# enoche/MMRec

Hardware: NVIDIA H100
Metric: graph-prop edges/sec (+ full-catalog scored-items/sec in extra) @ d=64 (higher is better)
Workload: dtype f32

## Files before the change

### mmrec_b200/csrc/score_cf.cu

```cuda
#include <climits>
#include <cstdio>
#include <cstdlib>

#include "batch_mask.cuh"
#include "select.cuh"
#include "tc_common.cuh"

namespace mmrec {

using namespace tc;

constexpr int CF_TILE = 128;
constexpr int CF_CONSUMER_WARPS = 8;
constexpr int CF_THREADS = 32 * CF_CONSUMER_WARPS + 32;
constexpr int CF_MAX_STAGES = 10;
constexpr int CF_CAP = 512;
constexpr int CF_EX_SLOTS = 128;
constexpr float CF_EPS = 1.125f / 1024.f;
constexpr float CF_EPS_SUB = 1.0f / 16777216.f;

struct CfSmem {
    uint32_t a, slab0, slab, bars, total;
    int stages;
};
__host__ __device__ inline CfSmem cf_smem(int KP) {
    CfSmem L;
    L.a = 0;
    L.slab0 = 2 * CF_TILE * KP * 2;
    const uint32_t slab = CF_TILE * KP * 2;
    L.slab = slab;
    L.stages = (int)((226u * 1024u - L.slab0 - 300u) / slab);
    if (L.stages > CF_MAX_STAGES) L.stages = CF_MAX_STAGES;
    L.bars = L.slab0 + L.stages * slab;
    L.total = L.bars + 32 * 8;
    return L;
}
enum { CB_AFULL = 0, CB_AFREE = 1, CB_FULL = 2, CB_EMPTY = 2 + CF_MAX_STAGES, CB_END = 2 + 2 * CF_MAX_STAGES };

struct CfParams {
    const char* Upk;
    const char* Ipk;
    int KP, n_it;
    int64_t B, n_items, n_units;
    float* gmax; int G, gw;
    const float* thr; uint4* bitmap;
    int dbg;
};

__device__ __forceinline__ void cf_producer(const CfParams& p, const CfSmem& L, uint32_t sbase, int64_t u0, int64_t u1) {
    const uint32_t bar = sbase + L.bars;
    const uint32_t a_bytes = 2 * CF_TILE * p.KP * 2;
    const uint32_t piece = L.slab < 16384u ? L.slab : 16384u;
    int64_t pair = u0 / p.n_it;
    int it = (int)(u0 - pair * p.n_it);
    bool new_pair = true;
    uint32_t a_cnt = 0, slot = 0, ph = 1;
    for (int64_t u = u0; u < u1; ++u) {
        if (new_pair) {
            if (a_cnt > 0) mbar_wait(bar + CB_AFREE * 8, (a_cnt - 1) & 1);
            mbar_expect_tx(bar + CB_AFULL * 8, a_bytes);
            const char* src = p.Upk + pair * (int64_t)a_bytes;
            for (uint32_t o = 0; o < a_bytes; o += 16384) bulk_g2s(sbase + L.a + o, src + o, 16384, bar + CB_AFULL * 8);
            ++a_cnt;
            new_pair = false;
        }
        const char* src = p.Ipk + (int64_t)it * L.slab;
        const uint32_t fb = bar + (CB_FULL + slot) * 8;
        mbar_wait(bar + (CB_EMPTY + slot) * 8, ph);
        if (p.dbg & 16) {
            mbar_arrive(fb);
        } else {
            mbar_expect_tx(fb, L.slab);
            const uint32_t dst = sbase + L.slab0 + slot * L.slab;
            for (uint32_t o = 0; o < L.slab; o += piece) bulk_g2s(dst + o, src + o, piece, fb);
        }
        if (++slot == (uint32_t)L.stages) { slot = 0; ph ^= 1; }
        if (++it == p.n_it) { it = 0; ++pair; new_pair = true; }
    }
}

template <int PASS, int GPT>
__device__ __forceinline__ void cf_consumer(const CfParams& p, const CfSmem& L, uint32_t sbase, int64_t u0, int64_t u1, int h) {
    const uint32_t bar = sbase + L.bars;
    constexpr uint32_t LBO = (CF_TILE / 8) * 128, SBO = 128;
    const int ksteps = p.KP / 16;
    const uint32_t half_bytes = CF_TILE * p.KP * 2;
    const int t = threadIdx.x & 127, w = t >> 5, lane = t & 31, q = lane & 3;
    const uint64_t a_desc0 = smem_desc(sbase + L.a + h * half_bytes, LBO, SBO), a_desc1 = smem_desc(sbase + L.a + h * half_bytes + 1024, LBO, SBO);
    const uint64_t b_desc0 = smem_desc(sbase + L.slab0, LBO, SBO);
    const uint64_t kstep = (2 * LBO) >> 4;
    const uint64_t slab_step = L.slab >> 4;
    float acc0[64], acc1[64];
#pragma unroll
    for (int i = 0; i < 64; ++i) { acc0[i] = 0.f; acc1[i] = 0.f; }
    int64_t pair = u0 / p.n_it;
    int it = (int)(u0 - pair * p.n_it);
    bool new_pair = true, live = false;
    uint32_t a_cnt = 0, slot = 0, ph = 0;
    uint64_t bd_slot = b_desc0;
    int64_t row0 = 0;
    float thr[4];
    for (int64_t u = u0; u < u1; ++u) {
        if (new_pair) {
            mbar_wait(bar + CB_AFULL * 8, a_cnt & 1);
            ++a_cnt;
            const int64_t base = pair * (2 * CF_TILE) + h * CF_TILE;
            live = base < p.B;
            row0 = base + 16 * w + (lane >> 2);
#pragma unroll
            for (int r = 0; r < 4; ++r) {
                const int64_t rr = row0 + 64 * (r >> 1) + 8 * (r & 1);
                if (PASS == 2) thr[r] = rr < p.B ? __ldg(p.thr + rr) : INFINITY;
            }
            new_pair = false;
        }
        mbar_wait(bar + (CB_FULL + slot) * 8, ph);
        if (live && !(p.dbg & 2)) {
            uint64_t ad0 = a_desc0, ad1 = a_desc1, bd = bd_slot;
            wgmma_fence();
#pragma unroll 4
            for (int j = 0; j < ksteps; ++j) {
                wgmma_f16<CF_TILE>(acc0, ad0, bd, j ? 1u : 0u);
                wgmma_f16<CF_TILE>(acc1, ad1, bd, j ? 1u : 0u);
                ad0 += kstep; ad1 += kstep; bd += kstep;
            }
            wgmma_commit();
            wgmma_wait<0>();
            wgmma_fence_regs(acc0);
            wgmma_fence_regs(acc1);
        }
        warp_arrive(bar + (CB_EMPTY + slot) * 8);
        bd_slot += slab_step;
        if (++slot == (uint32_t)L.stages) { slot = 0; ph ^= 1; bd_slot = b_desc0; }
        const int cur_it = it;
        if (++it == p.n_it) { it = 0; ++pair; new_pair = true; }
        if (new_pair || u + 1 == u1) warp_arrive(bar + CB_AFREE * 8);
        if (!live) continue;
        const int n_valid = (int)(p.n_items - (int64_t)cur_it * CF_TILE);
#pragma unroll
        for (int r = 0; r < 4; ++r) {
            const float* acc = r < 2 ? acc0 : acc1;
            const int e2 = r & 1;
            const int64_t row = row0 + 64 * (r >> 1) + 8 * e2;
            auto val = [&](int j, int e) {
                const float v = acc[4 * j + 2 * e2 + e];
                return 8 * j + 2 * q + e < n_valid ? v : -INFINITY;
            };
            if (PASS == 1) {
                group_max_store<GPT>(r < 2 ? acc0 : acc1, e2, q, n_valid, row, p.B, [&] { return p.gmax + row * p.G + (int64_t)cur_it * GPT; });
            } else {
                uint32_t wd[4] = {0u, 0u, 0u, 0u};
#pragma unroll
                for (int j = 0; j < 16; ++j)
#pragma unroll
                    for (int e = 0; e < 2; ++e)
                        if (!(__float_as_uint(val(j, e) - thr[r]) >> 31)) wd[j >> 2] |= 1u << (31 - (8 * (j & 3) + 2 * q + e));
#pragma unroll
                for (int b = 0; b < 4; ++b) {
                    wd[b] |= __shfl_xor_sync(0xffffffffu, wd[b], 1);
                    wd[b] |= __shfl_xor_sync(0xffffffffu, wd[b], 2);
                }
                if (q == r && row < p.B) p.bitmap[row * p.n_it + cur_it] = make_uint4(wd[0], wd[1], wd[2], wd[3]);
            }
        }
    }
}

template <int PASS, int GPT>
__global__ void __launch_bounds__(CF_THREADS, 1) cf_pass_kernel(const CfParams p) {
    extern __shared__ __align__(1024) uint8_t smem[];
    const CfSmem L = cf_smem(p.KP);
    const uint32_t sbase = smem_u32(smem);
    const int warp = threadIdx.x >> 5, lane = threadIdx.x & 31;
    const uint32_t bar = sbase + L.bars;
    if (threadIdx.x == 0) {
        mbar_init(bar + CB_AFULL * 8, 1);
        mbar_init(bar + CB_AFREE * 8, CF_CONSUMER_WARPS);
        for (int s = 0; s < CF_MAX_STAGES; ++s) {
            mbar_init(bar + (CB_FULL + s) * 8, 1);
            mbar_init(bar + (CB_EMPTY + s) * 8, CF_CONSUMER_WARPS);
        }
        mbar_fence_init();
    }
    __syncthreads();
    const int64_t u0 = (int64_t)blockIdx.x * p.n_units / gridDim.x;
    const int64_t u1 = (int64_t)(blockIdx.x + 1) * p.n_units / gridDim.x;
    if (warp == CF_CONSUMER_WARPS) {
        if (lane == 0) cf_producer(p, L, sbase, u0, u1);
    } else {
        cf_consumer<PASS, GPT>(p, L, sbase, u0, u1, warp >> 2);
    }
}

__device__ __forceinline__ void cf_pack_one(int64_t t, int64_t n_rows, const int64_t* __restrict__ idx, const float* __restrict__ E, int64_t ld,
                                            int d, int KP, const uint32_t* __restrict__ scale_src, uint4* __restrict__ out,
                                            float* __restrict__ row_norm, uint32_t* __restrict__ max_norm) {
    const int kblks = KP / 8;
    const int64_t row = t / kblks;
    const int kb = (int)(t % kblks);
    float x[8];
#pragma unroll
    for (int e = 0; e < 8; ++e) x[e] = 0.f;
    if (row < n_rows) {
        const float* src = E + (idx ? idx[row] : row) * ld;
#pragma unroll
        for (int e = 0; e < 8; ++e)
            if (kb * 8 + e < d) x[e] = __ldg(src + kb * 8 + e);
    }
    uint32_t am = 0u;
    if (!scale_src) {
#pragma unroll
        for (int e = 0; e < 8; ++e) { const uint32_t b = __float_as_uint(x[e]) & 0x7fffffffu; am = b > am ? b : am; }
        for (int o = kblks / 2; o > 0; o >>= 1) {
            const uint32_t a2 = __shfl_xor_sync(0xffffffffu, am, o);
            am = a2 > am ? a2 : am;
        }
    }
    const float sc = fp16_scale_for(scale_src ? __ldg(scale_src) : am);
    float ss = 0.f;
#pragma unroll
    for (int e = 0; e < 8; ++e) ss = fmaf(x[e] * sc, x[e] * sc, ss);
    for (int o = kblks / 2; o > 0; o >>= 1) ss += __shfl_xor_sync(0xffffffffu, ss, o);
    store_fp16x8(out, row / CF_TILE, kblks, kb, (int)(row % CF_TILE), x, sc);
    if (kb == 0 && row < n_rows) {
        const float nrm = sqrtf(ss) * (1.0f + 1e-6f);
        if (row_norm) row_norm[row] = nrm;
        if (max_norm) atomicMax(max_norm, __float_as_uint(nrm));
    }
}

__global__ void __launch_bounds__(256) cf_pack_items_kernel(int64_t n_items, const float* __restrict__ Ie, int64_t ldi, int d, int KP,
                                                            uint4* __restrict__ Ipk, uint32_t* __restrict__ header, int64_t n_threads) {
    const int64_t t = blockIdx.x * (int64_t)blockDim.x + threadIdx.x;
    if (t >= n_threads) return;
    if (t == 0) { header[1] = (uint32_t)n_items; header[2] = (uint32_t)d; header[3] = (uint32_t)KP; }
    cf_pack_one(t, n_items, nullptr, Ie, ldi, d, KP, header + 4, Ipk, nullptr, header);
}

__global__ void __launch_bounds__(256) cf_prep_kernel(int64_t mask_blocks, const BatchMask mask, int64_t nb, const int64_t* __restrict__ users,
                                                      const float* __restrict__ Ue, int64_t ldu, int d, int KP, uint4* __restrict__ Upk,
                                                      float* __restrict__ unorm, int64_t pack_threads, uint32_t* __restrict__ zero, int64_t zero_words) {
    if ((int64_t)blockIdx.x < mask_blocks) {
        mask_sorted_block(blockIdx.x, mask);
        return;
    }
    int64_t t = (blockIdx.x - mask_blocks) * (int64_t)blockDim.x + threadIdx.x;
    if (t < pack_threads) { cf_pack_one(t, nb, users, Ue, ldu, d, KP, nullptr, Upk, unorm, nullptr); return; }
    t -= pack_threads;
    if (t < zero_words) zero[t] = 0;
}

constexpr int CF_THR_BITS = 16;
template <int NV>
__device__ __forceinline__ uint32_t cf_warp_kth_coarse(const float* __restrict__ g, int G, int need, int lane) {
    uint32_t key[NV];
#pragma unroll
    for (int j = 0; j < NV; ++j) {
        const int t = j * 32 + lane;
        key[j] = t < G ? float_key(__ldg(g + t)) : 0u;
    }
    uint32_t kmax = 0u, kmin = 0xffffffffu;
#pragma unroll
    for (int j = 0; j < NV; ++j) {
        kmax = max(kmax, key[j]);
        if (j * 32 + lane < G && key[j] > 0x007fffffu) kmin = min(kmin, key[j]);
    }
    kmax = __reduce_max_sync(0xffffffffu, kmax);
    kmin = __reduce_min_sync(0xffffffffu, kmin);
    const int top = 31 - __clz((kmax ^ kmin) | (1u << (32 - CF_THR_BITS)));
    uint32_t prefix = top >= 31 ? 0u : (kmax & ~((2u << top) - 1u));
#pragma unroll 1
    for (int b = top; b >= 32 - CF_THR_BITS; --b) {
        const uint32_t cand = prefix | (1u << b);
// ... 496 lines not shown
```

### mmrec_b200/csrc/tc_common.cuh

```cuda
#pragma once
#include <cuda_fp16.h>

#include "common.cuh"
#include "wgmma.cuh"

namespace mmrec {
namespace tc {

__device__ __forceinline__ uint32_t smem_u32(const void* p) { return (uint32_t)__cvta_generic_to_shared(p); }

__device__ __forceinline__ void mbar_init(uint32_t bar, uint32_t count) {
    asm volatile("mbarrier.init.shared::cta.b64 [%0], %1;" ::"r"(bar), "r"(count) : "memory");
}
__device__ __forceinline__ void mbar_fence_init() { asm volatile("fence.mbarrier_init.release.cluster;" ::: "memory"); }
__device__ __forceinline__ void mbar_arrive(uint32_t bar) {
    asm volatile("mbarrier.arrive.shared::cta.b64 _, [%0];" ::"r"(bar) : "memory");
}
__device__ __forceinline__ void mbar_expect_tx(uint32_t bar, uint32_t bytes) {
    asm volatile("mbarrier.arrive.expect_tx.shared::cta.b64 _, [%0], %1;" ::"r"(bar), "r"(bytes) : "memory");
}
__device__ __forceinline__ bool mbar_try_wait(uint32_t bar, uint32_t parity) {
    uint32_t ok;
    asm volatile(
        "{\n\t.reg .pred p;\n\t"
        "mbarrier.try_wait.parity.shared::cta.b64 p, [%1], %2;\n\t"
        "selp.u32 %0, 1, 0, p;\n\t}"
        : "=r"(ok) : "r"(bar), "r"(parity) : "memory");
    return ok != 0;
}
__device__ __forceinline__ uint64_t global_ns() {
    uint64_t t;
    asm volatile("mov.u64 %0, %%globaltimer;" : "=l"(t));
    return t;
}
__device__ __forceinline__ void mbar_wait(uint32_t bar, uint32_t parity) {
    uint32_t spins = 0;
    uint64_t t0 = 0;
    while (!mbar_try_wait(bar, parity)) {
        if (++spins == 4096u) t0 = global_ns();
        if (spins > 4096u && (spins & 1023u) == 0 && global_ns() - t0 > 2000000000ull) __trap();
    }
}

__device__ __forceinline__ void bulk_g2s(uint32_t dst_smem, const void* src, uint32_t bytes, uint32_t bar) {
    asm volatile("cp.async.bulk.shared::cluster.global.mbarrier::complete_tx::bytes [%0], [%1], %2, [%3];"
                 ::"r"(dst_smem), "l"(src), "r"(bytes), "r"(bar) : "memory");
}

__device__ __forceinline__ void wgmma_fence() { asm volatile("wgmma.fence.sync.aligned;" ::: "memory"); }
__device__ __forceinline__ void wgmma_commit() { asm volatile("wgmma.commit_group.sync.aligned;" ::: "memory"); }
template <int N>
__device__ __forceinline__ void wgmma_wait() { asm volatile("wgmma.wait_group.sync.aligned %0;" ::"n"(N) : "memory"); }
template <int R>
__device__ __forceinline__ void wgmma_fence_regs(float (&d)[R]) {
#pragma unroll
    for (int i = 0; i < R; ++i) asm volatile("" : "+f"(d[i])::"memory");
}
__device__ __forceinline__ void fence_proxy_async() { asm volatile("fence.proxy.async.shared::cta;" ::: "memory"); }
__device__ __forceinline__ void warp_arrive(uint32_t bar) {
    __syncwarp();
    if ((threadIdx.x & 31) == 0) mbar_arrive(bar);
}

__device__ __forceinline__ uint64_t smem_desc(uint32_t smem_addr, uint32_t lbo_bytes, uint32_t sbo_bytes) {
    uint64_t d = 0;
    d |= (uint64_t)((smem_addr & 0x3FFFFu) >> 4);
    d |= (uint64_t)((lbo_bytes >> 4) & 0x3FFFu) << 16;
    d |= (uint64_t)((sbo_bytes >> 4) & 0x3FFFu) << 32;
    return d;
}

__device__ __forceinline__ void split_tf32(float x, float& hi, float& lo) {
    uint32_t h, l;
    asm("cvt.rna.tf32.f32 %0, %1;" : "=r"(h) : "f"(x));
    hi = __uint_as_float(h);
    asm("cvt.rna.tf32.f32 %0, %1;" : "=r"(l) : "f"(x - hi));
    lo = __uint_as_float(l);
}

__device__ __forceinline__ void split_tf32_trunc(float x, float& hi, float& lo) {
    hi = __uint_as_float(__float_as_uint(x) & 0xffffe000u);
    lo = x - hi;
}

}

__device__ __forceinline__ float fp16_scale_for(uint32_t m_bits) {
    const uint32_t e = (m_bits >> 23) & 0xffu;
    if (e == 0u || e == 255u || e < 14u) return 1.0f;
    return __uint_as_float((268u - e) << 23);
}

__global__ void absmax_norm_kernel(int64_t n, const float* __restrict__ X, int64_t ldx, int F, float* __restrict__ rnorm,
                                   uint32_t* __restrict__ amax, uint32_t* __restrict__ nmax);

__device__ __forceinline__ void store_fp16x8(uint4* __restrict__ out, int64_t tile, int kblks, int kb, int rr, const float (&x)[8], float sc) {
    uint32_t w[4];
#pragma unroll
    for (int e = 0; e < 4; ++e) {
        const __half2 h = __floats2half2_rn(x[2 * e] * sc, x[2 * e + 1] * sc);
        w[e] = *reinterpret_cast<const uint32_t*>(&h);
    }
    out[((tile * kblks + kb) * 16 + rr / 8) * 8 + (rr % 8)] = make_uint4(w[0], w[1], w[2], w[3]);
}

template <int GPT, class Dst>
__device__ __forceinline__ void group_max_store(const float (&acc)[64], int e2, int q, int n_valid, int64_t row, int64_t n_rows, Dst dst) {
    auto val = [&](int j, int e) { return 8 * j + 2 * q + e < n_valid ? acc[4 * j + 2 * e2 + e] : -INFINITY; };
    float gm[GPT];
#pragma unroll
    for (int g = 0; g < GPT; ++g) {
        float m = -INFINITY;
#pragma unroll
        for (int j = g * (16 / GPT); j < (g + 1) * (16 / GPT); ++j) m = fmaxf(m, fmaxf(val(j, 0), val(j, 1)));
        m = fmaxf(m, __shfl_xor_sync(0xffffffffu, m, 1));
        gm[g] = fmaxf(m, __shfl_xor_sync(0xffffffffu, m, 2));
    }
    if (row < n_rows) {
        float* d = dst();
#pragma unroll
        for (int g = 0; g < GPT; ++g)
            if ((g & 3) == q) d[g] = gm[g];
    }
}

__device__ __forceinline__ void set_threshold(float t, float margin, float* thr, int32_t* flag) {
    const bool finite = fabsf(t) < INFINITY && margin < INFINITY;
    *thr = finite ? t - margin : INFINITY;
    *flag = finite ? 0 : 2;
}

constexpr int TC_M = 128;
constexpr int TC_N = 256;
constexpr int TC_KC = 32;
constexpr int TC_SLAB_BYTES = TC_N * TC_KC * 4;
constexpr int TC_THREADS = 288;

template <int R>
__device__ __forceinline__ void pack_split_one(int64_t t, int64_t n_rows, const int64_t* __restrict__ idx, const float* __restrict__ E,
                                               int64_t ld, int d, int KP, float* __restrict__ hi, float* __restrict__ lo) {
    const int kblks = KP / 4;
    const int64_t row = t / kblks;
    const int kb = (int)(t % kblks);
    float x[4] = {0.f, 0.f, 0.f, 0.f};
    if (row < n_rows) {
        const float* src = E + (idx ? idx[row] : row) * ld;
#pragma unroll
        for (int e = 0; e < 4; ++e)
            if (kb * 4 + e < d) x[e] = __ldg(src + kb * 4 + e);
    }
    float4 h, l;
    tc::split_tf32(x[0], h.x, l.x); tc::split_tf32(x[1], h.y, l.y); tc::split_tf32(x[2], h.z, l.z); tc::split_tf32(x[3], h.w, l.w);
    const int64_t tile = row / R;
    const int rr = (int)(row % R);
    const int64_t off = ((tile * kblks + kb) * (R / 8) + rr / 8) * 32 + (rr % 8) * 4;
    *reinterpret_cast<float4*>(hi + off) = h;
    *reinterpret_cast<float4*>(lo + off) = l;
}

template <int R>
__global__ void pack_split_kernel(int64_t n_rows, const int64_t* __restrict__ idx, const float* __restrict__ E, int64_t ld,
                                  int d, int KP, float* __restrict__ hi, float* __restrict__ lo, int64_t n_tiles) {
    const int64_t t = blockIdx.x * (int64_t)blockDim.x + threadIdx.x;
    if (t >= n_tiles * R * (KP / 4)) return;
    pack_split_one<R>(t, n_rows, idx, E, ld, d, KP, hi, lo);
}

}
```

### mmrec_b200/csrc/spmm.cu

```cuda
#include <cooperative_groups.h>

#include "common.cuh"

namespace mmrec {

struct SpmmParams {
    int64_t n_rows, n_cols;
    const int32_t* rowptr; const int32_t* colidx; const float* vals;
    const int4* tasks; int64_t n_tasks, n_heavy; const int4* split_rows; int32_t* counters; float* partial;
    const float* X; int64_t ldx;
    float* Y; int64_t ldy;
    const float* acc_in; float* acc_out; int64_t ldacc; float acc_div;
    const float* gate_ref; int64_t ldgate;
    int y_acc;
    const float* post; int64_t post_row0; uint32_t spost;
    int d;
    uint32_t sx, sy, sacc, sgate;
    const float* X_hi; const float* acc_in_hi;
    int x_split, acc_split;
    uint32_t sx_hi, sacc_hi;
};


__device__ __forceinline__ const float4* row_f4(const float* base, uint32_t stride, int r, int f4) {
// ... 285 lines not shown

template <int D, int T>
__global__ void __launch_bounds__(256, VecCfg<D, T>::V == 1 ? 4 : 0) spmm_vec_kernel(const SpmmParams p) {
    __shared__ __align__(16) float red[(256 / T) * D];
    spmm_vec_body<D, T, false>(p, red);
}

template <int D, int T>
__global__ void __launch_bounds__(256) spmm_drop_kernel(const SpmmParams p, const uint32_t* __restrict__ keep, float scale) {
    __shared__ __align__(16) float red[(256 / T) * D];
    spmm_vec_body<D, T, false, true>(p, red, DropKeep{keep, scale});
}

__global__ void __launch_bounds__(256) edge_keep_bits_kernel(int64_t nnz, const float* __restrict__ draws, float keep_prob,
                                                             const int32_t* __restrict__ draw_of, const int32_t* __restrict__ mirror,
                                                             uint32_t* __restrict__ keep, uint32_t* __restrict__ keep_t) {
    const int64_t n_words = (nnz + 31) >> 5;
    const int lane = threadIdx.x & 31;
    const int64_t w0 = ((int64_t)blockIdx.x * blockDim.x + threadIdx.x) >> 5;
    const int64_t n_warps = ((int64_t)gridDim.x * blockDim.x) >> 5;
    auto kept = [&](int64_t e) { return floorf(__fadd_rn(keep_prob, __ldg(draws + __ldg(draw_of + e)))) != 0.f; };
    for (int64_t w = w0; w < n_words; w += n_warps) {
        const int64_t e = (w << 5) + lane;
        const bool in = e < nnz;
        const uint32_t word = __ballot_sync(0xffffffffu, in && kept(e));
        const uint32_t word_t = keep_t ? __ballot_sync(0xffffffffu, in && kept(__ldg(mirror + e))) : 0u;
        if (lane == 0) {
            keep[w] = word;
            if (keep_t) keep_t[w] = word_t;
        }
    }
}

constexpr int SPMM_CHAIN_MAX = 8;
struct SpmmChain { SpmmParams step[SPMM_CHAIN_MAX]; int n; unsigned sync_mask; };

template <int D, int T, bool COOP>
__global__ void __launch_bounds__(256, 3) spmm_chain_kernel(const SpmmChain c) {
    __shared__ __align__(16) float red[(256 / T) * D];
    for (int i = 0; i < c.n; ++i) {
        if (COOP && ((c.sync_mask >> i) & 1u)) { __threadfence(); cooperative_groups::this_grid().sync(); }
        spmm_vec_body<D, T, true>(c.step[i], red);
    }
}

__global__ void __launch_bounds__(256) spmm_generic_kernel(const SpmmParams p) {
    const int lane = threadIdx.x & 31;
    const int64_t warp0 = (int64_t)blockIdx.x * (blockDim.x >> 5) + (threadIdx.x >> 5);
    const int64_t nwarps = (int64_t)gridDim.x * (blockDim.x >> 5);
    for (int64_t row = warp0; row < p.n_rows; row += nwarps) {
        const int b = p.rowptr[row], e = p.rowptr[row + 1];
        float dot = 0.f, ny = 0.f, nr = 0.f;
        if (p.gate_ref) {
            for (int k0 = 0; k0 < p.d; k0 += 32) {
                const int k = k0 + lane;
                float acc = 0.f;
                if (k < p.d)
                    for (int j = b; j < e; ++j) acc = fmaf(p.vals[j], p.X[(int64_t)p.colidx[j] * p.ldx + k], acc);
                float r = k < p.d ? p.gate_ref[row * p.ldgate + k] : 0.f;
                dot += acc * r; ny += acc * acc; nr += r * r;
            }
            dot = warp_sum(dot); ny = warp_sum(ny); nr = warp_sum(nr);
        }
        const float c = p.gate_ref ? dot / (fmaxf(sqrtf(ny), 1e-8f) * fmaxf(sqrtf(nr), 1e-8f)) : 1.f;
        for (int k0 = 0; k0 < p.d; k0 += 32) {
            const int k = k0 + lane;
            if (k >= p.d) continue;
            float acc = 0.f;
            for (int j = b; j < e; ++j) acc = fmaf(p.vals[j], p.X[(int64_t)p.colidx[j] * p.ldx + k], acc);
            if (p.gate_ref) acc *= c;
            if (p.Y) p.Y[row * p.ldy + k] = p.y_acc ? p.Y[row * p.ldy + k] + acc : acc;
            if (p.acc_out) {
                float a = acc + (p.acc_in ? p.acc_in[row * p.ldacc + k] : 0.f);
                if (p.acc_div != 1.0f) a = __fdiv_rn(a, p.acc_div);
                if (p.post && row >= p.post_row0) a += p.post[(row - p.post_row0) * (int64_t)(p.spost / 4) + k];
                p.acc_out[row * p.ldacc + k] = a;
            }
        }
    }
}

int g_spmm_lanes = 0;

template <int D, int T, bool DROP = false>
static int launch_vec(const SpmmParams& p, cudaStream_t stream, const DropKeep dk = DropKeep{nullptr, 1.f}) {
    static int blocks_per_sm = 0;
    if (!blocks_per_sm) {
        if constexpr (DROP) MMREC_CUDA(cudaOccupancyMaxActiveBlocksPerMultiprocessor(&blocks_per_sm, spmm_drop_kernel<D, T>, 256, 0));
        else MMREC_CUDA(cudaOccupancyMaxActiveBlocksPerMultiprocessor(&blocks_per_sm, spmm_vec_kernel<D, T>, 256, 0));
        if (blocks_per_sm < 1) blocks_per_sm = 1;
    }
    const int64_t n_work = p.tasks ? p.n_tasks : p.n_rows;
    const int per_block = 8 * (32 / T);
    int64_t grid = (n_work - p.n_heavy + per_block - 1) / per_block;
    if (grid < p.n_heavy) grid = p.n_heavy;
    const int64_t cap = (int64_t)sm_count() * blocks_per_sm;
    if (grid > cap) grid = cap;
    if (grid < 1) return MMREC_OK;
    if constexpr (DROP) spmm_drop_kernel<D, T><<<(unsigned)grid, 256, 0, stream>>>(p, dk.keep, dk.scale);
    else spmm_vec_kernel<D, T><<<(unsigned)grid, 256, 0, stream>>>(p);
    MMREC_LAUNCH_CHECK();
    return MMREC_OK;
}

template <int D>
static int launch_vec_d(const SpmmParams& p, cudaStream_t stream) {
    constexpr int T4 = D / 4 > 32 ? 32 : D / 4;
    constexpr int T8 = D / 8 > 32 ? 32 : D / 8;
    constexpr int T16 = D / 16 > 32 ? 32 : D / 16;
    int T = g_spmm_lanes ? g_spmm_lanes : T4;
    if (T == T4) return launch_vec<D, T4>(p, stream);
    if (T == T16) return launch_vec<D, T16>(p, stream);
    return launch_vec<D, T8>(p, stream);
}

template <int D>
static int launch_vec_3d(const SpmmParams& p, cudaStream_t stream) {
    static_assert(VecCfg<D, D / 12>::V == 3, "three float4 per lane");
    return launch_vec<D, D / 12>(p, stream);
}

}

using namespace mmrec;

extern "C" int mmrec_spmm_set_lanes(int lanes_per_row) {
    MMREC_CHECK_ARG(lanes_per_row == 0 || lanes_per_row == 2 || lanes_per_row == 4 || lanes_per_row == 8 ||
                    lanes_per_row == 16 || lanes_per_row == 32, "spmm_set_lanes: 0 (default) or a power of two <= 32");
    g_spmm_lanes = lanes_per_row;
    return MMREC_OK;
}

extern "C" int mmrec_edge_keep_bits(int64_t nnz, const float* draws, float keep_prob, const int32_t* draw_of, const int32_t* mirror,
                                    uint32_t* keep_bits, uint32_t* keep_bits_t, void* stream_) {
    cudaStream_t stream = (cudaStream_t)stream_;
    MMREC_CHECK_ARG(nnz >= 0 && nnz < (1ll << 31), "edge_keep_bits: nnz out of range");
    if (nnz == 0) return MMREC_OK;
    MMREC_CHECK_ARG(draws && draw_of && keep_bits && (!keep_bits_t || mirror), "edge_keep_bits: null pointer");
    const int64_t n_words = (nnz + 31) / 32;
    int64_t grid = (n_words + 7) / 8;
    const int64_t cap = (int64_t)sm_count() * 16;
    if (grid > cap) grid = cap;
    edge_keep_bits_kernel<<<(unsigned)grid, 256, 0, stream>>>(nnz, draws, keep_prob, draw_of, mirror, keep_bits, keep_bits_t);
    MMREC_LAUNCH_CHECK();
    return MMREC_OK;
}

namespace mmrec {
template <int D, bool COOP>
static int launch_chain(const SpmmChain& c, cudaStream_t stream) {
    constexpr int T = D / 4 > 32 ? 32 : D / 4;
    static int blocks_per_sm = 0;
    if (!blocks_per_sm) {
        MMREC_CUDA(cudaOccupancyMaxActiveBlocksPerMultiprocessor(&blocks_per_sm, spmm_chain_kernel<D, T, COOP>, 256, 0));
        if (blocks_per_sm < 1) blocks_per_sm = 1;
    }
    int64_t max_work = 1;
    for (int i = 0; i < c.n; ++i) {
        const int64_t work = c.step[i].n_tasks > c.step[i].n_heavy ? c.step[i].n_tasks : c.step[i].n_heavy * 8;
        if (work > max_work) max_work = work;
    }
    const int per_block = 8 * (32 / T);
    int64_t grid = (max_work + per_block - 1) / per_block;
    const int64_t cap = (int64_t)sm_count() * blocks_per_sm;
    if (grid > cap) grid = cap;
    if (grid < 1) grid = 1;
    if (COOP) {
        void* args[] = {(void*)&c};
        MMREC_CUDA(cudaLaunchCooperativeKernel((const void*)spmm_chain_kernel<D, T, true>, dim3((unsigned)grid), dim3(256), args, 0, stream));
        ++g_launches;
    } else {
        spmm_chain_kernel<D, T, false><<<(unsigned)grid, 256, 0, stream>>>(c);
        MMREC_LAUNCH_CHECK();
    }
    return MMREC_OK;
}

template <int D>
static int launch_steps(const SpmmChain& c, int cooperative, cudaStream_t stream) {
    if (cooperative) return launch_chain<D, true>(c, stream);
    constexpr int T = D / 4 > 32 ? 32 : D / 4;
    for (int i = 0; i < c.n;) {
        int j = i + 1;
        while (j < c.n && !((c.sync_mask >> j) & 1u)) ++j;
        const SpmmParams& p = c.step[i];
        int rc;
        if (j == i + 1 && p.x_split == p.n_cols && p.acc_split == p.n_rows) {
            rc = launch_vec<D, T>(p, stream);
        } else {
            SpmmChain run;
            run.n = j - i; run.sync_mask = 0;
            for (int k = 0; k < run.n; ++k) run.step[k] = c.step[i + k];
            rc = launch_chain<D, false>(run, stream);
        }
        if (rc != MMREC_OK) return rc;
        i = j;
    }
    return MMREC_OK;
}

static int spmm_op_params(const mmrec_spmm_op& o, int i, int d, bool chain, SpmmParams& p, bool& vec_ok) {
    MMREC_CHECK_ARG(o.n_rows >= 0 && o.n_cols >= 0 && o.rowptr && o.X && (o.Y || o.acc_out), "spmm: op %d: null pointer / bad sizes", i);
    MMREC_CHECK_ARG(o.tasks ? (o.n_tasks >= 0 && o.n_cta_tasks >= 0 && o.n_cta_tasks <= o.n_tasks && o.split_rows && o.counters && o.partial)
                            : !chain,
                    "spmm: op %d: work plan pointers missing (the chained kernel needs the plan of mmrec_spmm_plan)", i);
    MMREC_CHECK_ARG(o.ldx >= d && (!o.Y || o.ldy >= d) && (!o.acc_out || o.ldacc >= d) && (!o.gate_ref || o.ldgate >= d) &&
                    (!o.post || o.ldpost >= d) && o.acc_div != 0.0f, "spmm: op %d: leading dimension < d or acc_div == 0", i);
    MMREC_CHECK_ARG(!(o.y_accumulate && o.gate_ref), "spmm: y_accumulate does not combine with the cosine gate");
    MMREC_CHECK_ARG(o.ldx < (1ll << 30) && o.ldy < (1ll << 30) && o.ldacc < (1ll << 30) && o.ldgate < (1ll << 30) && o.ldpost < (1ll << 30) &&
                    o.n_cols < (1ll << 31) && o.n_rows < (1ll << 31), "spmm: op %d: leading dimension / size out of range", i);
    MMREC_CHECK_ARG(!o.X_hi || (o.x_split >= 0 && o.x_split <= o.n_cols && o.ldx_hi >= d && o.ldx_hi < (1ll << 30)),
                    "spmm: op %d: X_hi needs 0 <= x_split <= n_cols and d <= ldx_hi < 2^30", i);
    MMREC_CHECK_ARG(!o.acc_in_hi || (o.acc_in && o.acc_out && o.acc_in_split >= 0 && o.acc_in_split <= o.n_rows && o.ldacc_in_hi >= d &&
                                     o.ldacc_in_hi < (1ll << 30)),
                    "spmm: op %d: acc_in_hi needs acc_in, acc_out, 0 <= acc_in_split <= n_rows and d <= ldacc_in_hi < 2^30", i);
    p.n_rows = o.n_rows; p.n_cols = o.n_cols; p.rowptr = o.rowptr; p.colidx = o.colidx; p.vals = o.vals;
    p.tasks = (const int4*)o.tasks; p.n_tasks = o.n_tasks; p.n_heavy = o.tasks ? o.n_cta_tasks : 0; p.split_rows = (const int4*)o.split_rows;
    p.counters = o.counters; p.partial = o.partial; p.X = o.X; p.ldx = o.ldx; p.Y = o.Y; p.ldy = o.ldy; p.y_acc = o.y_accumulate != 0;
    p.acc_in = o.acc_in; p.acc_out = o.acc_out; p.ldacc = o.ldacc; p.acc_div = o.acc_div; p.gate_ref = o.gate_ref; p.ldgate = o.ldgate;
    p.post = o.post; p.post_row0 = o.post_row0; p.d = d;
    p.sx = (uint32_t)(o.ldx * 4); p.sy = (uint32_t)(o.ldy * 4); p.sacc = (uint32_t)(o.ldacc * 4); p.sgate = (uint32_t)(o.ldgate * 4);
    p.spost = (uint32_t)(o.ldpost * 4);
    p.X_hi = o.X_hi ? o.X_hi : o.X;
    p.x_split = (int)(o.X_hi ? o.x_split : o.n_cols);
    p.sx_hi = (uint32_t)((o.X_hi ? o.ldx_hi : o.ldx) * 4);
    p.acc_in_hi = o.acc_in_hi ? o.acc_in_hi : o.acc_in;
    p.acc_split = (int)(o.acc_in_hi ? o.acc_in_split : o.n_rows);
    p.sacc_hi = (uint32_t)((o.acc_in_hi ? o.ldacc_in_hi : o.ldacc) * 4);
    auto al16 = [](const void* q, int64_t ld) { return q == nullptr || ((((uintptr_t)q) & 15) == 0 && (ld & 3) == 0); };
    vec_ok = al16(o.X, o.ldx) && al16(o.Y, o.ldy) && al16(o.acc_in, o.ldacc) && al16(o.acc_out, o.ldacc) && al16(o.gate_ref, o.ldgate) &&
             al16(o.post, o.ldpost) && al16(o.partial, 4) && al16(o.X_hi, o.ldx_hi) && al16(o.acc_in_hi, o.ldacc_in_hi);
    return MMREC_OK;
}
}

extern "C" int mmrec_spmm_run_f32(int d, int n_ops, const mmrec_spmm_op* ops, int cooperative, void* stream_) {
    cudaStream_t stream = (cudaStream_t)stream_;
    MMREC_CHECK_ARG(n_ops >= 1 && n_ops <= SPMM_CHAIN_MAX && ops, "spmm: 1 <= n_ops <= %d", SPMM_CHAIN_MAX);
// ... 77 lines not shown
```

Baseline: 15.06 billion.

## Software-pipeline CF scoring wgmma with epilogue and specialize k-steps at compile time

The consumer loop in the CF scoring kernel is restructured so that the wgmma for the second half-tile (and the next slab's first half) runs while the epilogue for the previous accumulator executes, instead of waiting for all MMAs before the masking/bitmap work. The k-step count becomes a template parameter so the MMA loop fully unrolls, and index arithmetic is narrowed to 32-bit ints. The GPT==8 group-max store is vectorized into a float2 write. Dead tiles beyond B are no longer skipped for MMA, and the primary graph-propagation metric does not exercise this kernel.

```diff
diff --git a/mmrec_b200/csrc/score_cf.cu b/mmrec_b200/csrc/score_cf.cu
--- a/mmrec_b200/csrc/score_cf.cu
+++ b/mmrec_b200/csrc/score_cf.cu
@@ -79,11 +79,10 @@
     }
 }
 
-template <int PASS, int GPT>
+template <int PASS, int GPT, int KS>
 __device__ __forceinline__ void cf_consumer(const CfParams& p, const CfSmem& L, uint32_t sbase, int64_t u0, int64_t u1, int h) {
     const uint32_t bar = sbase + L.bars;
     constexpr uint32_t LBO = (CF_TILE / 8) * 128, SBO = 128;
-    const int ksteps = p.KP / 16;
     const uint32_t half_bytes = CF_TILE * p.KP * 2;
     const int t = threadIdx.x & 127, w = t >> 5, lane = t & 31, q = lane & 3;
     const uint64_t a_desc0 = smem_desc(sbase + L.a + h * half_bytes, LBO, SBO), a_desc1 = smem_desc(sbase + L.a + h * half_bytes + 1024, LBO, SBO);
@@ -93,76 +92,82 @@
     float acc0[64], acc1[64];
 #pragma unroll
     for (int i = 0; i < 64; ++i) { acc0[i] = 0.f; acc1[i] = 0.f; }
-    int64_t pair = u0 / p.n_it;
-    int it = (int)(u0 - pair * p.n_it);
-    bool new_pair = true, live = false;
+    int pair = (int)(u0 / p.n_it);
+    int it = (int)(u0 - (int64_t)pair * p.n_it);
     uint32_t a_cnt = 0, slot = 0, ph = 0;
     uint64_t bd_slot = b_desc0;
-    int64_t row0 = 0;
-    float thr[4];
-    for (int64_t u = u0; u < u1; ++u) {
-        if (new_pair) {
-            mbar_wait(bar + CB_AFULL * 8, a_cnt & 1);
-            ++a_cnt;
-            const int64_t base = pair * (2 * CF_TILE) + h * CF_TILE;
-            live = base < p.B;
-            row0 = base + 16 * w + (lane >> 2);
-#pragma unroll
-            for (int r = 0; r < 4; ++r) {
-                const int64_t rr = row0 + 64 * (r >> 1) + 8 * (r & 1);
-                if (PASS == 2) thr[r] = rr < p.B ? __ldg(p.thr + rr) : INFINITY;
+    int row0 = 0;
+    auto issue = [&](float (&acc)[64], uint64_t ad, uint64_t bd) {
+        wgmma_fence();
+#pragma unroll
+        for (int j = 0; j < KS; ++j) {
+            wgmma_f16<CF_TILE>(acc, ad, bd, j ? 1u : 0u);
+            ad += kstep; bd += kstep;
+        }
+        wgmma_commit();
+    };
+    auto start_pair = [&] {
+        mbar_wait(bar + CB_AFULL * 8, a_cnt & 1);
+        ++a_cnt;
+        const int base = pair * (2 * CF_TILE) + h * CF_TILE;
+        row0 = base + 16 * w + (lane >> 2);
+        mbar_wait(bar + (CB_FULL + slot) * 8, ph);
+        issue(acc0, a_desc0, bd_slot);
+    };
+    auto epilogue = [&](const float (&acc)[64], int r, int cur_it, int n_valid) {
+        const int e2 = r & 1;
+        const int row = row0 + 64 * (r >> 1) + 8 * e2;
+        auto val = [&](int j, int e) {
+            const float v = acc[4 * j + 2 * e2 + e];
+            return 8 * j + 2 * q + e < n_valid ? v : -INFINITY;
+        };
+        if (PASS == 1) {
+            group_max_store<GPT>(acc, e2, q, n_valid, row, p.B, [&] { return p.gmax + (int64_t)row * p.G + cur_it * GPT; });
+        } else {
+            const float thr = row < p.B ? __ldg(p.thr + row) : INFINITY;
+            uint32_t wd[4] = {0u, 0u, 0u, 0u};
+#pragma unroll
+            for (int j = 0; j < 16; ++j)
+#pragma unroll
+                for (int e = 0; e < 2; ++e)
+                    if (!(__float_as_uint(val(j, e) - thr) >> 31)) wd[j >> 2] |= 1u << (31 - (8 * (j & 3) + 2 * q + e));
+#pragma unroll
+            for (int b = 0; b < 4; ++b) {
+                wd[b] |= __shfl_xor_sync(0xffffffffu, wd[b], 1);
+                wd[b] |= __shfl_xor_sync(0xffffffffu, wd[b], 2);
             }
-            new_pair = false;
-        }
-        mbar_wait(bar + (CB_FULL + slot) * 8, ph);
-        if (live && !(p.dbg & 2)) {
-            uint64_t ad0 = a_desc0, ad1 = a_desc1, bd = bd_slot;
-            wgmma_fence();
-#pragma unroll 4
-            for (int j = 0; j < ksteps; ++j) {
-                wgmma_f16<CF_TILE>(acc0, ad0, bd, j ? 1u : 0u);
-                wgmma_f16<CF_TILE>(acc1, ad1, bd, j ? 1u : 0u);
-                ad0 += kstep; ad1 += kstep; bd += kstep;
-            }
-            wgmma_commit();
-            wgmma_wait<0>();
-            wgmma_fence_regs(acc0);
-            wgmma_fence_regs(acc1);
-        }
-        warp_arrive(bar + (CB_EMPTY + slot) * 8);
+            if (q == r && row < p.B) p.bitmap[(int64_t)row * p.n_it + cur_it] = make_uint4(wd[0], wd[1], wd[2], wd[3]);
+        }
+    };
+    int left = (int)(u1 - u0);
+    if (left > 0) start_pair();
+    for (; left > 0; --left) {
+        issue(acc1, a_desc1, bd_slot);
+        wgmma_wait<1>();
+        wgmma_fence_regs(acc0);
+        const int cur_it = it;
+        const int n_valid = (int)(p.n_items - (int64_t)cur_it * CF_TILE);
+        epilogue(acc0, 0, cur_it, n_valid);
+        epilogue(acc0, 1, cur_it, n_valid);
+        const uint32_t done = slot;
         bd_slot += slab_step;
         if (++slot == (uint32_t)L.stages) { slot = 0; ph ^= 1; bd_slot = b_desc0; }
-        const int cur_it = it;
+        bool new_pair = false;
         if (++it == p.n_it) { it = 0; ++pair; new_pair = true; }
-        if (new_pair || u + 1 == u1) warp_arrive(bar + CB_AFREE * 8);
-        if (!live) continue;
-        const int n_valid = (int)(p.n_items - (int64_t)cur_it * CF_TILE);
-#pragma unroll
-        for (int r = 0; r < 4; ++r) {
-            const float* acc = r < 2 ? acc0 : acc1;
-            const int e2 = r & 1;
-            const int64_t row = row0 + 64 * (r >> 1) + 8 * e2;
-            auto val = [&](int j, int e) {
-                const float v = acc[4 * j + 2 * e2 + e];
-                return 8 * j + 2 * q + e < n_valid ? v : -INFINITY;
-            };
-            if (PASS == 1) {
-                group_max_store<GPT>(r < 2 ? acc0 : acc1, e2, q, n_valid, row, p.B, [&] { return p.gmax + row * p.G + (int64_t)cur_it * GPT; });
-            } else {
-                uint32_t wd[4] = {0u, 0u, 0u, 0u};
-#pragma unroll
-                for (int j = 0; j < 16; ++j)
-#pragma unroll
-                    for (int e = 0; e < 2; ++e)
-                        if (!(__float_as_uint(val(j, e) - thr[r]) >> 31)) wd[j >> 2] |= 1u << (31 - (8 * (j & 3) + 2 * q + e));
-#pragma unroll
-                for (int b = 0; b < 4; ++b) {
-                    wd[b] |= __shfl_xor_sync(0xffffffffu, wd[b], 1);
-                    wd[b] |= __shfl_xor_sync(0xffffffffu, wd[b], 2);
-                }
-                if (q == r && row < p.B) p.bitmap[row * p.n_it + cur_it] = make_uint4(wd[0], wd[1], wd[2], wd[3]);
-            }
-        }
+        const bool ahead = !new_pair && left > 1;
+        if (ahead) {
+            mbar_wait(bar + (CB_FULL + slot) * 8, ph);
+            issue(acc0, a_desc0, bd_slot);
+            wgmma_wait<1>();
+        } else {
+            wgmma_wait<0>();
+        }
+        wgmma_fence_regs(acc1);
+        warp_arrive(bar + (CB_EMPTY + done) * 8);
+        if (!ahead) warp_arrive(bar + CB_AFREE * 8);
+        epilogue(acc1, 2, cur_it, n_valid);
+        epilogue(acc1, 3, cur_it, n_valid);
+        if (new_pair && left > 1) start_pair();
     }
 }
 
@@ -171,7 +176,7 @@
     extern __shared__ __align__(1024) uint8_t smem[];
     const CfSmem L = cf_smem(p.KP);
     const uint32_t sbase = smem_u32(smem);
-    const int warp = threadIdx.x >> 5, lane = threadIdx.x & 31;
+    const int warp = __shfl_sync(0xffffffffu, (int)(threadIdx.x >> 5), 0), lane = threadIdx.x & 31;
     const uint32_t bar = sbase + L.bars;
     if (threadIdx.x == 0) {
         mbar_init(bar + CB_AFULL * 8, 1);
@@ -188,7 +193,13 @@
     if (warp == CF_CONSUMER_WARPS) {
         if (lane == 0) cf_producer(p, L, sbase, u0, u1);
     } else {
-        cf_consumer<PASS, GPT>(p, L, sbase, u0, u1, warp >> 2);
+        const int h = warp >> 2;
+        switch ((p.dbg & 2) ? 0 : p.KP / 16) {
+            case 0: cf_consumer<PASS, GPT, 0>(p, L, sbase, u0, u1, h); break;
+            case 2: cf_consumer<PASS, GPT, 2>(p, L, sbase, u0, u1, h); break;
+            case 4: cf_consumer<PASS, GPT, 4>(p, L, sbase, u0, u1, h); break;
+            default: cf_consumer<PASS, GPT, 8>(p, L, sbase, u0, u1, h); break;
+        }
     }
 }
 
diff --git a/mmrec_b200/csrc/tc_common.cuh b/mmrec_b200/csrc/tc_common.cuh
--- a/mmrec_b200/csrc/tc_common.cuh
+++ b/mmrec_b200/csrc/tc_common.cuh
@@ -118,9 +118,15 @@
     }
     if (row < n_rows) {
         float* d = dst();
+        if constexpr (GPT == 8) {
+            const float lo = q == 0 ? gm[0] : (q == 1 ? gm[2] : (q == 2 ? gm[4] : gm[6]));
+            const float hi = q == 0 ? gm[1] : (q == 1 ? gm[3] : (q == 2 ? gm[5] : gm[7]));
+            *reinterpret_cast<float2*>(d + 2 * q) = make_float2(lo, hi);
+        } else {
 #pragma unroll
-        for (int g = 0; g < GPT; ++g)
-            if ((g & 3) == q) d[g] = gm[g];
+            for (int g = 0; g < GPT; ++g)
+                if ((g & 3) == q) d[g] = gm[g];
+        }
     }
 }
 
```

Measured after the change: 15.10 billion (median of 6 runs). About the same (+0.2%).

## Split CF consumers into 16 single-accumulator warps with register reallocation and quad-scatter reductions

Applied to the files above, without the earlier changes.

The scoring kernel now runs 16 consumer warps, each warpgroup holding one 64-row accumulator instead of two. Producer warps shrink their register budget with setmaxnreg so consumers get more. Tail masking is applied only on the last item tile, the hit bitmap and group-max use recursive-halving quad shuffles that write one word per lane, and the K-loop is specialized at compile time. Separately, the SpMM launches set the shared-memory carveout to prefer L1, which mainly targets the graph-prop edges/sec metric, and the change adds occupancy probing at first launch.

```diff
diff --git a/mmrec_b200/csrc/score_cf.cu b/mmrec_b200/csrc/score_cf.cu
--- a/mmrec_b200/csrc/score_cf.cu
+++ b/mmrec_b200/csrc/score_cf.cu
@@ -1,6 +1,7 @@
 #include <climits>
 #include <cstdio>
 #include <cstdlib>
+#include <type_traits>
 
 #include "batch_mask.cuh"
 #include "select.cuh"
@@ -11,8 +12,9 @@
 using namespace tc;
 
 constexpr int CF_TILE = 128;
-constexpr int CF_CONSUMER_WARPS = 8;
-constexpr int CF_THREADS = 32 * CF_CONSUMER_WARPS + 32;
+constexpr int CF_CONSUMER_WARPS = 16;
+constexpr int CF_THREADS = 32 * CF_CONSUMER_WARPS + 128;
+constexpr int CF_PRODUCER_REGS = 32, CF_CONSUMER_REGS = 112;
 constexpr int CF_MAX_STAGES = 10;
 constexpr int CF_CAP = 512;
 constexpr int CF_EX_SLOTS = 128;
@@ -79,55 +81,73 @@
     }
 }
 
+__device__ __forceinline__ uint32_t cf_hit_word(const float (&acc)[64], int e2, int q, float thr) {
+    uint32_t wd[4];
+#pragma unroll
+    for (int b = 0; b < 4; ++b) {
+        uint32_t s[2] = {0u, 0u};
+#pragma unroll
+        for (int jj = 0; jj < 4; ++jj)
+#pragma unroll
+            for (int e = 0; e < 2; ++e) {
+                const float v = acc[4 * (4 * b + jj) + 2 * e2 + e];
+                s[e] = __funnelshift_l(__float_as_uint(v - thr), s[e], 8);
+            }
+        wd[b] = ((~s[0] & 0x80808080u) | ((~s[1] & 0x80808080u) >> 1)) >> (2 * q);
+    }
+    auto bit_or = [](uint32_t a, uint32_t b) { return a | b; };
+    quad_scatter_step<2, 4>(wd, q, bit_or);
+    quad_scatter_step<1, 2>(wd, q, bit_or);
+    return wd[0];
+}
+
 template <int PASS, int GPT>
-__device__ __forceinline__ void cf_consumer(const CfParams& p, const CfSmem& L, uint32_t sbase, int64_t u0, int64_t u1, int h) {
+__device__ __forceinline__ void cf_consumer(const CfParams& p, const CfSmem& L, uint32_t sbase, int64_t u0, int64_t u1, int g) {
     const uint32_t bar = sbase + L.bars;
     constexpr uint32_t LBO = (CF_TILE / 8) * 128, SBO = 128;
-    const int ksteps = p.KP / 16;
-    const uint32_t half_bytes = CF_TILE * p.KP * 2;
     const int t = threadIdx.x & 127, w = t >> 5, lane = t & 31, q = lane & 3;
-    const uint64_t a_desc0 = smem_desc(sbase + L.a + h * half_bytes, LBO, SBO), a_desc1 = smem_desc(sbase + L.a + h * half_bytes + 1024, LBO, SBO);
+    const uint64_t a_desc = smem_desc(sbase + L.a + (g >> 1) * (CF_TILE * p.KP * 2) + (g & 1) * 1024, LBO, SBO);
     const uint64_t b_desc0 = smem_desc(sbase + L.slab0, LBO, SBO);
     const uint64_t kstep = (2 * LBO) >> 4;
     const uint64_t slab_step = L.slab >> 4;
-    float acc0[64], acc1[64];
-#pragma unroll
-    for (int i = 0; i < 64; ++i) { acc0[i] = 0.f; acc1[i] = 0.f; }
+    float acc[64];
+#pragma unroll
+    for (int i = 0; i < 64; ++i) acc[i] = 0.f;
     int64_t pair = u0 / p.n_it;
     int it = (int)(u0 - pair * p.n_it);
     bool new_pair = true, live = false;
     uint32_t a_cnt = 0, slot = 0, ph = 0;
     uint64_t bd_slot = b_desc0;
-    int64_t row0 = 0;
-    float thr[4];
+    const int nb = (int)p.B;
+    int row0 = 0;
+    float thr[2];
+    const int last_valid = (int)(p.n_items - (int64_t)(p.n_it - 1) * CF_TILE);
     for (int64_t u = u0; u < u1; ++u) {
         if (new_pair) {
             mbar_wait(bar + CB_AFULL * 8, a_cnt & 1);
             ++a_cnt;
-            const int64_t base = pair * (2 * CF_TILE) + h * CF_TILE;
-            live = base < p.B;
+            const int base = (int)pair * (2 * CF_TILE) + g * 64;
+            live = base < nb;
             row0 = base + 16 * w + (lane >> 2);
 #pragma unroll
-            for (int r = 0; r < 4; ++r) {
-                const int64_t rr = row0 + 64 * (r >> 1) + 8 * (r & 1);
-                if (PASS == 2) thr[r] = rr < p.B ? __ldg(p.thr + rr) : INFINITY;
-            }
+            for (int e2 = 0; e2 < 2; ++e2)
+                if (PASS == 2) thr[e2] = row0 + 8 * e2 < nb ? __ldg(p.thr + row0 + 8 * e2) : INFINITY;
             new_pair = false;
         }
         mbar_wait(bar + (CB_FULL + slot) * 8, ph);
         if (live && !(p.dbg & 2)) {
-            uint64_t ad0 = a_desc0, ad1 = a_desc1, bd = bd_slot;
-            wgmma_fence();
-#pragma unroll 4
-            for (int j = 0; j < ksteps; ++j) {
-                wgmma_f16<CF_TILE>(acc0, ad0, bd, j ? 1u : 0u);
-                wgmma_f16<CF_TILE>(acc1, ad1, bd, j ? 1u : 0u);
-                ad0 += kstep; ad1 += kstep; bd += kstep;
-            }
-            wgmma_commit();
-            wgmma_wait<0>();
-            wgmma_fence_regs(acc0);
-            wgmma_fence_regs(acc1);
+            auto mmas = [&](auto ks) {
+                wgmma_fence();
+                wgmma_f16<CF_TILE>(acc, a_desc, bd_slot, 0u);
+#pragma unroll
+                for (int j = 1; j < decltype(ks)::value; ++j) wgmma_f16<CF_TILE>(acc, a_desc + j * kstep, bd_slot + j * kstep, 1u);
+                wgmma_commit();
+                wgmma_wait<0>();
+                wgmma_fence_regs(acc);
+            };
+            if (p.KP == 32) mmas(std::integral_constant<int, 2>());
+            else if (p.KP == 64) mmas(std::integral_constant<int, 4>());
+            else mmas(std::integral_constant<int, 8>());
         }
         warp_arrive(bar + (CB_EMPTY + slot) * 8);
         bd_slot += slab_step;
@@ -136,31 +156,20 @@
         if (++it == p.n_it) { it = 0; ++pair; new_pair = true; }
         if (new_pair || u + 1 == u1) warp_arrive(bar + CB_AFREE * 8);
         if (!live) continue;
-        const int n_valid = (int)(p.n_items - (int64_t)cur_it * CF_TILE);
-#pragma unroll
-        for (int r = 0; r < 4; ++r) {
-            const float* acc = r < 2 ? acc0 : acc1;
-            const int e2 = r & 1;
-            const int64_t row = row0 + 64 * (r >> 1) + 8 * e2;
-            auto val = [&](int j, int e) {
-                const float v = acc[4 * j + 2 * e2 + e];
-                return 8 * j + 2 * q + e < n_valid ? v : -INFINITY;
-            };
+        if (cur_it + 1 == p.n_it && last_valid < CF_TILE) {
+#pragma unroll
+            for (int i = 0; i < 64; ++i)
+                if (8 * (i >> 2) + 2 * q + (i & 1) >= last_valid) acc[i] = -INFINITY;
+        }
+#pragma unroll
+        for (int e2 = 0; e2 < 2; ++e2) {
+            const int row = row0 + 8 * e2;
             if (PASS == 1) {
-                group_max_store<GPT>(r < 2 ? acc0 : acc1, e2, q, n_valid, row, p.B, [&] { return p.gmax + row * p.G + (int64_t)cur_it * GPT; });
+                group_max_store<GPT>(acc, e2, q, std::integral_constant<int, CF_TILE>(), row, nb,
+                                     [&] { return p.gmax + (row * p.G + cur_it * GPT); });
             } else {
-                uint32_t wd[4] = {0u, 0u, 0u, 0u};
-#pragma unroll
-                for (int j = 0; j < 16; ++j)
-#pragma unroll
-                    for (int e = 0; e < 2; ++e)
-                        if (!(__float_as_uint(val(j, e) - thr[r]) >> 31)) wd[j >> 2] |= 1u << (31 - (8 * (j & 3) + 2 * q + e));
-#pragma unroll
-                for (int b = 0; b < 4; ++b) {
-                    wd[b] |= __shfl_xor_sync(0xffffffffu, wd[b], 1);
-                    wd[b] |= __shfl_xor_sync(0xffffffffu, wd[b], 2);
-                }
-                if (q == r && row < p.B) p.bitmap[row * p.n_it + cur_it] = make_uint4(wd[0], wd[1], wd[2], wd[3]);
+                const uint32_t wd = cf_hit_word(acc, e2, q, thr[e2]);
+                if (row < nb) reinterpret_cast<uint32_t*>(p.bitmap + (row * p.n_it + cur_it))[q] = wd;
             }
         }
     }
@@ -185,9 +194,11 @@
     __syncthreads();
     const int64_t u0 = (int64_t)blockIdx.x * p.n_units / gridDim.x;
     const int64_t u1 = (int64_t)(blockIdx.x + 1) * p.n_units / gridDim.x;
-    if (warp == CF_CONSUMER_WARPS) {
-        if (lane == 0) cf_producer(p, L, sbase, u0, u1);
+    if (warp >= CF_CONSUMER_WARPS) {
+        asm volatile("setmaxnreg.dec.sync.aligned.u32 %0;\n" ::"n"(CF_PRODUCER_REGS) : "memory");
+        if (warp == CF_CONSUMER_WARPS && lane == 0) cf_producer(p, L, sbase, u0, u1);
     } else {
+        asm volatile("setmaxnreg.inc.sync.aligned.u32 %0;\n" ::"n"(CF_CONSUMER_REGS) : "memory");
         cf_consumer<PASS, GPT>(p, L, sbase, u0, u1, warp >> 2);
     }
 }
diff --git a/mmrec_b200/csrc/spmm.cu b/mmrec_b200/csrc/spmm.cu
--- a/mmrec_b200/csrc/spmm.cu
+++ b/mmrec_b200/csrc/spmm.cu
@@ -391,13 +391,33 @@
 
 int g_spmm_lanes = 0;
 
+static int occupancy_prefer_l1(const void* f) {
+    int blocks = 0;
+    MMREC_CUDA(cudaOccupancyMaxActiveBlocksPerMultiprocessor(&blocks, f, 256, 0));
+    cudaFuncAttributes a;
+    MMREC_CUDA(cudaFuncGetAttributes(&a, f));
+    int dev = 0, smem_sm = 0;
+    MMREC_CUDA(cudaGetDevice(&dev));
+    MMREC_CUDA(cudaDeviceGetAttribute(&smem_sm, cudaDevAttrMaxSharedMemoryPerMultiprocessor, dev));
+    if (blocks < 1 || smem_sm <= 0) return blocks < 1 ? 1 : blocks;
+    const int64_t need = (int64_t)blocks * ((int64_t)a.sharedSizeBytes + 1024);
+    const int pct = (int)((need * 100 + smem_sm - 1) / smem_sm);
+    MMREC_CUDA(cudaFuncSetAttribute(f, cudaFuncAttributePreferredSharedMemoryCarveout, pct < 1 ? 1 : pct));
+    int after = 0;
+    MMREC_CUDA(cudaOccupancyMaxActiveBlocksPerMultiprocessor(&after, f, 256, 0));
+    if (after < blocks) MMREC_CUDA(cudaFuncSetAttribute(f, cudaFuncAttributePreferredSharedMemoryCarveout, cudaSharedmemCarveoutDefault));
+    return blocks;
+}
+
 template <int D, int T, bool DROP = false>
 static int launch_vec(const SpmmParams& p, cudaStream_t stream, const DropKeep dk = DropKeep{nullptr, 1.f}) {
     static int blocks_per_sm = 0;
     if (!blocks_per_sm) {
-        if constexpr (DROP) MMREC_CUDA(cudaOccupancyMaxActiveBlocksPerMultiprocessor(&blocks_per_sm, spmm_drop_kernel<D, T>, 256, 0));
-        else MMREC_CUDA(cudaOccupancyMaxActiveBlocksPerMultiprocessor(&blocks_per_sm, spmm_vec_kernel<D, T>, 256, 0));
-        if (blocks_per_sm < 1) blocks_per_sm = 1;
+        int b;
+        if constexpr (DROP) b = occupancy_prefer_l1((const void*)spmm_drop_kernel<D, T>);
+        else b = occupancy_prefer_l1((const void*)spmm_vec_kernel<D, T>);
+        if (b < 0) return b;
+        blocks_per_sm = b;
     }
     const int64_t n_work = p.tasks ? p.n_tasks : p.n_rows;
     const int per_block = 8 * (32 / T);
@@ -461,8 +481,9 @@
     constexpr int T = D / 4 > 32 ? 32 : D / 4;
     static int blocks_per_sm = 0;
     if (!blocks_per_sm) {
-        MMREC_CUDA(cudaOccupancyMaxActiveBlocksPerMultiprocessor(&blocks_per_sm, spmm_chain_kernel<D, T, COOP>, 256, 0));
-        if (blocks_per_sm < 1) blocks_per_sm = 1;
+        const int b = occupancy_prefer_l1((const void*)spmm_chain_kernel<D, T, COOP>);
+        if (b < 0) return b;
+        blocks_per_sm = b;
     }
     int64_t max_work = 1;
     for (int i = 0; i < c.n; ++i) {
diff --git a/mmrec_b200/csrc/tc_common.cuh b/mmrec_b200/csrc/tc_common.cuh
--- a/mmrec_b200/csrc/tc_common.cuh
+++ b/mmrec_b200/csrc/tc_common.cuh
@@ -104,23 +104,46 @@
     out[((tile * kblks + kb) * 16 + rr / 8) * 8 + (rr % 8)] = make_uint4(w[0], w[1], w[2], w[3]);
 }
 
-template <int GPT, class Dst>
-__device__ __forceinline__ void group_max_store(const float (&acc)[64], int e2, int q, int n_valid, int64_t row, int64_t n_rows, Dst dst) {
+template <int O, int N, class T, class Op>
+__device__ __forceinline__ void quad_scatter_step(T* x, int q, Op op) {
+    const bool up = (q & O) != 0;
+#pragma unroll
+    for (int i = 0; i < N / 2; ++i) {
+        const T keep = up ? x[i + N / 2] : x[i], send = up ? x[i] : x[i + N / 2];
+        x[i] = op(keep, __shfl_xor_sync(0xffffffffu, send, O));
+    }
+}
+
+template <int GPT, class Dst, class NV>
+__device__ __forceinline__ void group_max_store(const float (&acc)[64], int e2, int q, NV n_valid, int64_t row, int64_t n_rows, Dst dst) {
     auto val = [&](int j, int e) { return 8 * j + 2 * q + e < n_valid ? acc[4 * j + 2 * e2 + e] : -INFINITY; };
+    auto mx = [](float a, float b) { return fmaxf(a, b); };
     float gm[GPT];
 #pragma unroll
     for (int g = 0; g < GPT; ++g) {
         float m = -INFINITY;
 #pragma unroll
         for (int j = g * (16 / GPT); j < (g + 1) * (16 / GPT); ++j) m = fmaxf(m, fmaxf(val(j, 0), val(j, 1)));
-        m = fmaxf(m, __shfl_xor_sync(0xffffffffu, m, 1));
-        gm[g] = fmaxf(m, __shfl_xor_sync(0xffffffffu, m, 2));
+        gm[GPT >= 4 ? (g & 3) * (GPT / 4) + g / 4 : g] = m;
+    }
+    if constexpr (GPT >= 4) {
+        quad_scatter_step<2, GPT>(gm, q, mx);
+        quad_scatter_step<1, GPT / 2>(gm, q, mx);
+    } else if constexpr (GPT == 2) {
+        quad_scatter_step<1, 2>(gm, q, mx);
+        gm[0] = fmaxf(gm[0], __shfl_xor_sync(0xffffffffu, gm[0], 2));
+    } else {
+        gm[0] = fmaxf(gm[0], __shfl_xor_sync(0xffffffffu, gm[0], 1));
+        gm[0] = fmaxf(gm[0], __shfl_xor_sync(0xffffffffu, gm[0], 2));
     }
     if (row < n_rows) {
         float* d = dst();
+        if constexpr (GPT >= 4) {
 #pragma unroll
-        for (int g = 0; g < GPT; ++g)
-            if ((g & 3) == q) d[g] = gm[g];
+            for (int i = 0; i < GPT / 4; ++i) d[q + 4 * i] = gm[i];
+        } else if (q < GPT) {
+            d[q] = gm[0];
+        }
     }
 }
 
```

Result: no change. 15.01 billion before, 15.17 billion after (median of 6 runs) (+1.1%).
